# AHupuJR/REFID

Measured on AMD Instinct MI355X. Metric: interpolated frames/sec (train step) GoPro 256x256 11+1, higher is better.
Workload: dtype f32

## Files before the change

### refid_amd/csrc/conv_pw.hip

```cpp
#include "common.h"
#include "conv_args.h"
#include "conv_epilogue.h"
#include "conv_planes.h"
#include <cstdlib>

namespace {

typedef unsigned int u32x4 __attribute__((ext_vector_type(4)));
constexpr int KC = 8;
__device__ constexpr int PW_TA[6] = {0, 1, 0, 2, 0, 1};
__device__ constexpr int PW_TB[6] = {0, 0, 1, 0, 2, 1};

template <int NT, int XD, bool EX, bool SIX = false>
__global__ __launch_bounds__(256, (SIX || NT > 2) ? 3 : 4) void conv_pw_kernel(const ConvKArgs a, const PwExtra e) {
    const int lane = threadIdx.x & 63, wave = threadIdx.x >> 6;
    const int li = lane & 31, kh = lane >> 5;
    const long long npix = (long long)a.N * a.H * a.W;
    const long long p0 = ((long long)blockIdx.x * 4 + wave) * 32;
    const long long p = p0 + li;
    const int n0 = blockIdx.y * (32 * NT);

    const long long spanA = a.patchW ? (npix / a.patchW) * (long long)a.patchRow : npix * a.ldA;
    const long long spanB = a.patchW ? spanA - a.patchRow / 2 : npix * (a.inB ? a.ldB : a.ldA);
    const __amdgpu_buffer_rsrc_t rsA = __builtin_amdgcn_make_buffer_rsrc(
        const_cast<float*>(a.inA), 0, (int)min(spanA * 4, 0x7fffffffLL), 0x00020000);
    const __amdgpu_buffer_rsrc_t rsB = __builtin_amdgcn_make_buffer_rsrc(
        const_cast<float*>(a.inB ? a.inB : a.inA), 0, (int)min(spanB * 4, 0x7fffffffLL), 0x00020000);
    const __amdgpu_buffer_rsrc_t rsW = __builtin_amdgcn_make_buffer_rsrc(
        const_cast<float*>(a.w), 0, (int)min((long long)a.nchunks * a.CoutPad * KC * (SIX ? 6 : 4), 0x7fffffffLL), 0x00020000);
    const bool pok = p < npix;
    const long long pA = a.patchW ? (p / a.patchW) * a.patchRow + (p % a.patchW) * a.ldA : p * a.ldA;
    const long long pB = a.patchW ? (p / a.patchW) * a.patchRow + (p % a.patchW) * a.ldB : p * a.ldB;
    const int voA = pok ? (int)(pA * 4) + kh * 16 : OOB;
    const int voB = pok ? (int)(pB * 4) + kh * 16 : OOB;
    int voW[NT];
#pragma unroll
    for (int nt = 0; nt < NT; ++nt) {
        const int row = a.coBase + n0 + nt * 32 + li;
        voW[nt] = (row < a.CoutPad) ? (SIX ? row * 32 + kh * 16 : (row * KC + kh * 4) * 4) : OOB;
    }
    const int wChunk = a.CoutPad * KC * 4;
    const int wPlane = a.CoutPad * 32;

    f32x16 acc[NT];
#pragma unroll
    for (int nt = 0; nt < NT; ++nt)
#pragma unroll
        for (int r = 0; r < 16; ++r) acc[nt][r] = 0.f;

    auto load_x = [&](int ch) -> f32x4 {
        const int c0 = ch * KC;
        const bool fromA = c0 < a.Ca;
        const int soff = (fromA ? c0 : c0 - a.Ca) * 4;
        const int vo = (c0 + kh * 4 < a.Ctot) ? (fromA ? voA : voB) : OOB;
        const u32x4 v = fromA ? __builtin_amdgcn_raw_buffer_load_b128(rsA, vo, soff, 0)
                              : __builtin_amdgcn_raw_buffer_load_b128(rsB, vo, soff, 0);
        return __builtin_bit_cast(f32x4, v);
    };
    auto load_w = [&](int ch, f32x4 (&dst)[NT]) {
#pragma unroll
        for (int nt = 0; nt < NT; ++nt)
            dst[nt] = __builtin_bit_cast(f32x4, __builtin_amdgcn_raw_buffer_load_b128(rsW, voW[nt], ch * wChunk, 0));
    };
    auto load_w6 = [&](int c16, f32x4 (&dst)[3][NT]) {
#pragma unroll
        for (int pl = 0; pl < 3; ++pl)
#pragma unroll
            for (int nt = 0; nt < NT; ++nt)
                dst[pl][nt] = __builtin_bit_cast(f32x4, __builtin_amdgcn_raw_buffer_load_b128(rsW, voW[nt], (c16 * 3 + pl) * wPlane, 0));
    };
    auto mfma6 = [&](const f32x4& x0, const f32x4& x1, const f32x4 (&w6)[3][NT]) {
        f32x4 pl[3];
        split8<3>(x0, x1, pl);
#pragma unroll
        for (int t = 0; t < 6; ++t)
#pragma unroll
            for (int nt = 0; nt < NT; ++nt)
                acc[nt] = __builtin_amdgcn_mfma_f32_32x32x16_bf16(__builtin_bit_cast(bf16x8, w6[PW_TA[t]][nt]),
                                                                  __builtin_bit_cast(bf16x8, pl[PW_TB[t]]), acc[nt], 0, 0, 0);
    };

    f32x4 xr[2 * XD];
    f32x4 wr[SIX ? 1 : 2][NT];
    f32x4 w6[SIX ? 2 : 1][3][NT];
    const int nch = a.nchunks;
    __shared__ float sS[EX ? 128 : 1];
    bool ln_done = false;
    if constexpr (EX) {
        if (e.pool != nullptr) {
            __shared__ float sM[128], sZ[64];
            const int C = e.seC, Ch = C / 2, tid = threadIdx.x;
            const int n = (int)(((long long)blockIdx.x * 128) / e.hw);
            for (int c = tid; c < C; c += 256) {
                const float* pp = e.pool + (long long)n * e.poolParts * C + c;
                float s0 = 0.f;
                for (int r = 0; r < e.poolParts; ++r) s0 += pp[(long long)r * C];
                sM[c] = s0 * e.invHW;
            }
            __syncthreads();
            for (int j = tid; j < Ch; j += 256) {
                float z = e.seB1[j];
                for (int c = 0; c < C; ++c) z += e.seW1[j * C + c] * sM[c];
                sZ[j] = z > 0.f ? z : 0.f;
            }
            __syncthreads();
            for (int c = tid; c < C; c += 256) {
                float v = e.seB2[c];
                for (int j = 0; j < Ch; ++j) v += e.seW2[c * Ch + j] * sZ[j];
                sS[c] = 1.f / (1.f + __expf(-v));
            }
            __syncthreads();
            if (e.seS != nullptr && blockIdx.y == 0 && ((long long)blockIdx.x * 128) % e.hw == 0) {
                for (int c = tid; c < C; c += 256) { e.seM[n * C + c] = sM[c]; e.seS[n * C + c] = sS[c]; }
                for (int j = tid; j < Ch; j += 256) e.seZ1[n * Ch + j] = sZ[j];
            }
        }
        if (e.lnG != nullptr) {
#pragma unroll
            for (int j = 0; j < 2 * XD; ++j) xr[j] = (j < nch) ? load_x(j) : f32x4{0.f, 0.f, 0.f, 0.f};
            if constexpr (SIX) load_w6(0, w6[0]);
            else load_w(0, wr[0]);
            float s1 = 0.f;
#pragma unroll
            for (int j = 0; j < 2 * XD; ++j) s1 += (xr[j][0] + xr[j][1]) + (xr[j][2] + xr[j][3]);
            s1 += __shfl_xor(s1, 32, 64);
            const float mu = s1 / (float)a.Ctot;
            float s2 = 0.f;
#pragma unroll
            for (int j = 0; j < 2 * XD; ++j)
                if (j < nch) {
#pragma unroll
                    for (int k = 0; k < 4; ++k) { const float d = xr[j][k] - mu; s2 += d * d; }
                }
            s2 += __shfl_xor(s2, 32, 64);
            const float rstd = 1.f / sqrtf(s2 / (float)a.Ctot + e.lnEps);
#pragma unroll
            for (int j = 0; j < 2 * XD; ++j)
                if (j < nch) {
                    const int c = j * KC + kh * 4;
                    const f32x4 gv = *reinterpret_cast<const f32x4*>(e.lnG + c);
                    const f32x4 bv = *reinterpret_cast<const f32x4*>(e.lnB + c);
#pragma unroll
                    for (int k = 0; k < 4; ++k) xr[j][k] = (xr[j][k] - mu) * rstd * gv[k] + bv[k];
                    if (e.lnOut != nullptr && blockIdx.y == 0 && pok)
                        *reinterpret_cast<f32x4*>(e.lnOut + p * e.ldLn + c) = xr[j];
                }
            if constexpr (SIX) {
#pragma unroll
                for (int j = 0; j < 2 * XD; j += 2)
                    if (j < nch) {
                        if (j + 2 < nch) load_w6(j / 2 + 1, w6[(j / 2 + 1) & 1]);
                        mfma6(xr[j], xr[j + 1], w6[(j / 2) & 1]);
                    }
            } else {
#pragma unroll
                for (int j = 0; j < 2 * XD; ++j)
                    if (j < nch) {
                        if (j + 1 < nch) load_w(j + 1, wr[(j + 1) & 1]);
#pragma unroll
                        for (int kk = 0; kk < 4; ++kk)
#pragma unroll
                            for (int nt = 0; nt < NT; ++nt)
                                acc[nt] = __builtin_amdgcn_mfma_f32_32x32x2f32(wr[j & 1][nt][kk], xr[j][kk], acc[nt], 0, 0, 0);
                    }
            }
            ln_done = true;
        }
    }
    if (!ln_done) {
#pragma unroll
        for (int j = 0; j < XD; ++j)
            if (j < nch) xr[j] = load_x(j);
        if constexpr (SIX) load_w6(0, w6[0]);
        else load_w(0, wr[0]);
        for (int c0 = 0; c0 < nch; c0 += 2 * XD) {
#pragma unroll
            for (int j = 0; j < 2 * XD; ++j) {
                const int c = c0 + j;
                if (c < nch) {
                    if constexpr (SIX) {
                        if ((j & 1) == 0 && c + 2 < nch) load_w6(c / 2 + 1, w6[(j / 2 + 1) & 1]);
                    } else {
                        if (c + 1 < nch) load_w(c + 1, wr[(j + 1) & 1]);
                    }
                    if (c + XD < nch) xr[(j + XD) % (2 * XD)] = load_x(c + XD);
                    if constexpr (EX) {
                        if (e.pool != nullptr) {
                            const int k0 = c * KC + kh * 4;
                            const f32x4 sv = *reinterpret_cast<const f32x4*>(&sS[k0 % e.seC]);
                            xr[j] *= sv;
                            if (e.xsOut != nullptr && blockIdx.y == 0 && pok)
                                *reinterpret_cast<f32x4*>(e.xsOut + p * e.ldXs + k0) = xr[j];
                        }
                    }
                    if constexpr (SIX) {
                        if (j & 1) mfma6(xr[j - 1], xr[j], w6[(j / 2) & 1]);
                    } else {
#pragma unroll
                        for (int kk = 0; kk < 4; ++kk)
#pragma unroll
                            for (int nt = 0; nt < NT; ++nt)
                                acc[nt] = __builtin_amdgcn_mfma_f32_32x32x2f32(wr[j & 1][nt][kk], xr[j][kk], acc[nt], 0, 0, 0);
                    }
                }
            }
        }
    }

    if (a.vecOK) {
        constexpr int HN = (NT > 2) ? 2 : NT;
        constexpr int PITCH = 8 * HN + 1;
        __shared__ f32x4 sT[4][32 * PITCH];
        f32x4* t = sT[wave];
#pragma unroll
        for (int h0 = 0; h0 < NT; h0 += HN) {
            if (h0) __syncthreads();
#pragma unroll
            for (int nt = 0; nt < HN; ++nt)
#pragma unroll
                for (int g = 0; g < 4; ++g) {
                    f32x4 v;
#pragma unroll
                    for (int k = 0; k < 4; ++k) v[k] = acc[h0 + nt][4 * g + k];
                    t[li * PITCH + nt * 8 + 2 * g + kh] = v;
                }
            __syncthreads();
#pragma unroll
            for (int it = 0; it < 4 * HN; ++it) {
                const int f = it * 64 + lane;
                const int px = f / (8 * HN), c4 = f % (8 * HN);
                const long long pp = p0 + px;
                const int j0 = n0 + h0 * 32 + c4 * 4;
                if (pp >= npix || j0 >= a.Cout) continue;
                f32x4 v = t[px * PITCH + c4];
                if (a.shuffle) {
                    const int Co1 = a.Cout >> 2;
                    const unsigned qd = (unsigned)j0 / (unsigned)Co1, ch = (unsigned)j0 - qd * Co1;
                    const unsigned up = (unsigned)pp, row = up / (unsigned)a.W, x = up - row * a.W;
                    const long long op = (long long)(2 * row + (qd >> 1)) * (2 * a.W) + 2 * x + (qd & 1);
                    conv_epilogue(a, v, ch, j0, true, EpiAtOp{op, (int)ch}, false);
                    continue;
                }
                const float* res2 = nullptr;
                if constexpr (EX) {
                    if (e.res2) res2 = e.res2 + pp * e.ldR2 + j0;
                }
                conv_epilogue<true>(a, v, a.coBase + j0, j0, true, EpiAtOp{pp, j0}, false, res2);
                if constexpr (EX) {
                    if (e.out2) {
                        f32x4 gl;
#pragma unroll
                        for (int k = 0; k < 4; ++k) gl[k] = gelu_f(v[k]);
                        *reinterpret_cast<f32x4*>(e.out2 + pp * e.ldO2 + j0) = gl;
                    }
                }
            }
        }
        return;
    }
    if (!pok) return;
#pragma unroll
    for (int nt = 0; nt < NT; ++nt) {
#pragma unroll
        for (int g = 0; g < 4; ++g) {
            const int j0 = n0 + nt * 32 + 8 * g + 4 * kh;
            f32x4 v;
#pragma unroll
            for (int k = 0; k < 4; ++k) v[k] = acc[nt][4 * g + k];
            conv_epilogue<true>(a, v, a.coBase + j0, j0, false, EpiAtOp{p, j0});
        }
    }
}

}

int refid_launch_pointwise(const ConvKArgs& ka, hipStream_t st, const PwExtra* ex, int terms) {
    ConvKArgs a = ka;
    a.nchunks = cdiv(a.Ctot, KC);
    if (a.Cout % 4) a.vecOK = 0;
    const long long npix = (long long)a.N * a.H * a.W;
    const int nb = (int)((npix + 127) / 128);
    const bool six = terms == 6;
    REFID_CHECK(!a.shuffle || (a.vecOK && ex == nullptr && terms == 0 && a.mask == nullptr && a.Cout > 32 && (a.Cout / 4) % 4 == 0 &&
                               npix < 0x7fffffffLL),
                "conv2d: ConvTranspose2d on the pointwise tile needs 16-byte aligned tensors, fp32 products, no mask / fusions and "
                "at least 16 output channels");
    REFID_CHECK(a.out2 == nullptr || (a.vecOK && ex == nullptr), "conv2d: the pointwise tile's second output needs 16-byte aligned tensors and no fusions");
    REFID_CHECK(!a.patchW || (terms == 0 && ex == nullptr && a.inB != nullptr), "conv2d: the patch form of the pointwise tile has fp32 products, no fusions");
    REFID_CHECK(terms == 0 || terms == 6, "conv2d: the pointwise tile has fp32 products (0) or six bf16 products (6), got %d", terms);
    REFID_CHECK(!six || (a.Ctot % 16 == 0 && (a.inB == nullptr || a.Ca % 16 == 0) && a.Cout > 32),
                "conv2d: the six-product pointwise tile needs channel counts that are multiples of 16 and more than 32 outputs");
    if (ex != nullptr) {
        REFID_CHECK(a.vecOK && a.Cout > 32, "conv2d: pointwise fusions need 16-byte aligned tensors and more than 32 outputs");
        REFID_CHECK(!ex->lnG || (a.inB == nullptr && a.Ctot % 8 == 0 && a.Ctot <= 64 && ex->lnB),
                    "conv2d: the LayerNorm prologue needs one source of at most 64 channels (got %d)", a.Ctot);
        REFID_CHECK(!ex->pool || (ex->hw > 0 && ex->hw % 128 == 0 && ex->seC >= 8 && ex->seC <= 128 && ex->seC % 8 == 0 &&
                                  a.Ctot % ex->seC == 0 && ex->poolParts > 0 && ex->seW1 && ex->seB1 && ex->seW2 && ex->seB2 &&
                                  (!ex->seS || (ex->seM && ex->seZ1)) && !ex->lnG),
                    "conv2d: bad squeeze-excite fusion arguments (pixels per sample must be a multiple of 128)");
        if (six) hipLaunchKernelGGL((conv_pw_kernel<2, 4, true, true>), dim3(nb, cdiv(a.Cout, 64)), dim3(256), 0, st, a, *ex);
        else hipLaunchKernelGGL((conv_pw_kernel<2, 4, true>), dim3(nb, cdiv(a.Cout, 64)), dim3(256), 0, st, a, *ex);
        REFID_LAUNCH_CHECK("conv_pw/fused");
        return 0;
    }
    const PwExtra none;
    if (six) hipLaunchKernelGGL((conv_pw_kernel<2, 4, false, true>), dim3(nb, cdiv(a.Cout, 64)), dim3(256), 0, st, a, none);
    else if (a.Cout <= 32) hipLaunchKernelGGL((conv_pw_kernel<1, 8, false>), dim3(nb, 1), dim3(256), 0, st, a, none);
    else {
        static const bool nt4 = []() { const char* e = getenv("REFID_PW_NT4"); return e && e[0] == '1'; }();
        if (nt4 && a.Cout % 128 == 0)
            hipLaunchKernelGGL((conv_pw_kernel<4, 4, false>), dim3(nb, a.Cout / 128), dim3(256), 0, st, a, none);
        else
            hipLaunchKernelGGL((conv_pw_kernel<2, 4, false>), dim3(nb, cdiv(a.Cout, 64)), dim3(256), 0, st, a, none);
    }
    REFID_LAUNCH_CHECK("conv_pw");
    return 0;
}
```

Baseline: 545.6.

## Remap pointwise conv grid for XCD locality and use wave-local swizzled transpose epilogue

Replaces the 2D grid with a 1D grid whose block index is decoded so that consecutive pixel blocks land on the same XCD and all column tiles of a pixel block are adjacent. The shared-memory transpose in the epilogue now uses an XOR swizzle instead of padding, and it synchronises with a wave barrier instead of block-wide __syncthreads, since each wave only touches its own slab. Bias is hoisted into a register before the main loop, and per-item output addresses are computed incrementally through EpiSteps. It drops the NT4 environment variant, and it relies on a new ncot field and new helpers that live elsewhere.

```diff
diff --git a/refid_amd/csrc/conv_pw.hip b/refid_amd/csrc/conv_pw.hip
--- a/refid_amd/csrc/conv_pw.hip
+++ b/refid_amd/csrc/conv_pw.hip
@@ -2,7 +2,6 @@
 #include "conv_args.h"
 #include "conv_epilogue.h"
 #include "conv_planes.h"
-#include <cstdlib>
 
 namespace {
 
@@ -12,13 +11,19 @@
 __device__ constexpr int PW_TB[6] = {0, 0, 1, 0, 2, 1};
 
 template <int NT, int XD, bool EX, bool SIX = false>
-__global__ __launch_bounds__(256, (SIX || NT > 2) ? 3 : 4) void conv_pw_kernel(const ConvKArgs a, const PwExtra e) {
+__global__ __launch_bounds__(256, SIX ? 3 : 4) void conv_pw_kernel(const ConvKArgs a, const PwExtra e) {
+    static_assert(NT == 1 || NT == 2, "the transpose slab holds the wave's whole column tile in one pass");
     const int lane = threadIdx.x & 63, wave = threadIdx.x >> 6;
     const int li = lane & 31, kh = lane >> 5;
     const long long npix = (long long)a.N * a.H * a.W;
-    const long long p0 = ((long long)blockIdx.x * 4 + wave) * 32;
+    const int xcd = blockIdx.x & 7, slot = blockIdx.x >> 3;
+    const int pb = (slot / a.ncot) * 8 + xcd;
+    const long long wg0 = (long long)pb * 128;
+    if (wg0 >= npix) return;
+    const int ct = slot % a.ncot;
+    const int n0 = ct * (32 * NT);
+    const long long p0 = wg0 + wave * 32;
     const long long p = p0 + li;
-    const int n0 = blockIdx.y * (32 * NT);
 
     const long long spanA = a.patchW ? (npix / a.patchW) * (long long)a.patchRow : npix * a.ldA;
     const long long spanB = a.patchW ? spanA - a.patchRow / 2 : npix * (a.inB ? a.ldB : a.ldA);
@@ -41,6 +46,9 @@
     }
     const int wChunk = a.CoutPad * KC * 4;
     const int wPlane = a.CoutPad * 32;
+    const int c4 = lane % (8 * NT), j0 = n0 + c4 * 4;
+    f32x4 bq = {0.f, 0.f, 0.f, 0.f};
+    if (a.vecOK && a.bias && !a.shuffle && j0 < a.Cout) bq = epi_load4(a.bias + a.coBase + j0);
 
     f32x16 acc[NT];
 #pragma unroll
@@ -90,7 +98,7 @@
         if (e.pool != nullptr) {
             __shared__ float sM[128], sZ[64];
             const int C = e.seC, Ch = C / 2, tid = threadIdx.x;
-            const int n = (int)(((long long)blockIdx.x * 128) / e.hw);
+            const int n = (int)(wg0 / e.hw);
             for (int c = tid; c < C; c += 256) {
                 const float* pp = e.pool + (long long)n * e.poolParts * C + c;
                 float s0 = 0.f;
@@ -110,7 +118,7 @@
                 sS[c] = 1.f / (1.f + __expf(-v));
             }
             __syncthreads();
-            if (e.seS != nullptr && blockIdx.y == 0 && ((long long)blockIdx.x * 128) % e.hw == 0) {
+            if (e.seS != nullptr && ct == 0 && wg0 % e.hw == 0) {
                 for (int c = tid; c < C; c += 256) { e.seM[n * C + c] = sM[c]; e.seS[n * C + c] = sS[c]; }
                 for (int j = tid; j < Ch; j += 256) e.seZ1[n * Ch + j] = sZ[j];
             }
@@ -142,7 +150,7 @@
                     const f32x4 bv = *reinterpret_cast<const f32x4*>(e.lnB + c);
 #pragma unroll
                     for (int k = 0; k < 4; ++k) xr[j][k] = (xr[j][k] - mu) * rstd * gv[k] + bv[k];
-                    if (e.lnOut != nullptr && blockIdx.y == 0 && pok)
+                    if (e.lnOut != nullptr && ct == 0 && pok)
                         *reinterpret_cast<f32x4*>(e.lnOut + p * e.ldLn + c) = xr[j];
                 }
             if constexpr (SIX) {
@@ -189,7 +197,7 @@
                             const int k0 = c * KC + kh * 4;
                             const f32x4 sv = *reinterpret_cast<const f32x4*>(&sS[k0 % e.seC]);
                             xr[j] *= sv;
-                            if (e.xsOut != nullptr && blockIdx.y == 0 && pok)
+                            if (e.xsOut != nullptr && ct == 0 && pok)
                                 *reinterpret_cast<f32x4*>(e.xsOut + p * e.ldXs + k0) = xr[j];
                         }
                     }
@@ -208,52 +216,56 @@
     }
 
     if (a.vecOK) {
-        constexpr int HN = (NT > 2) ? 2 : NT;
-        constexpr int PITCH = 8 * HN + 1;
+        constexpr int PITCH = 8 * NT;
         __shared__ f32x4 sT[4][32 * PITCH];
         f32x4* t = sT[wave];
 #pragma unroll
-        for (int h0 = 0; h0 < NT; h0 += HN) {
-            if (h0) __syncthreads();
-#pragma unroll
-            for (int nt = 0; nt < HN; ++nt)
-#pragma unroll
-                for (int g = 0; g < 4; ++g) {
-                    f32x4 v;
-#pragma unroll
-                    for (int k = 0; k < 4; ++k) v[k] = acc[h0 + nt][4 * g + k];
-                    t[li * PITCH + nt * 8 + 2 * g + kh] = v;
+        for (int nt = 0; nt < NT; ++nt)
+#pragma unroll
+            for (int g = 0; g < 4; ++g) {
+                f32x4 v;
+#pragma unroll
+                for (int k = 0; k < 4; ++k) v[k] = acc[nt][4 * g + k];
+                t[li * PITCH + ((nt * 8 + 2 * g + kh) ^ (li & 7))] = v;
+            }
+        __builtin_amdgcn_fence(__ATOMIC_RELEASE, "wavefront");
+        __builtin_amdgcn_wave_barrier();
+        __builtin_amdgcn_fence(__ATOMIC_ACQUIRE, "wavefront");
+        constexpr int PPI = 8 / NT, ITEMS = 4 * NT;
+        const int px0 = lane / (8 * NT);
+        if (j0 >= a.Cout) return;
+        const EpiSteps epi(a, a.out, p0 + px0, j0, PPI, 0, true);
+        const float* res2 = nullptr;
+        float* gout2 = nullptr;
+        int res2Step = 0, gout2Step = 0;
+        if constexpr (EX) {
+            if (e.res2) { res2 = e.res2 + (p0 + px0) * e.ldR2 + j0; res2Step = PPI * e.ldR2; }
+            if (e.out2) { gout2 = e.out2 + (p0 + px0) * e.ldO2 + j0; gout2Step = PPI * e.ldO2; }
+        }
+#pragma unroll
+        for (int it = 0; it < ITEMS; ++it) {
+            const int px = it * PPI + px0;
+            const long long pp = p0 + px;
+            if (pp >= npix) continue;
+            f32x4 v = t[px * PITCH + (c4 ^ (px & 7))];
+            if (a.shuffle) {
+                const int Co1 = a.Cout >> 2;
+                const unsigned qd = (unsigned)j0 / (unsigned)Co1, ch = (unsigned)j0 - qd * Co1;
+                const unsigned up = (unsigned)pp, row = up / (unsigned)a.W, x = up - row * a.W;
+                const long long op = (long long)(2 * row + (qd >> 1)) * (2 * a.W) + 2 * x + (qd & 1);
+                conv_epilogue(a, v, ch, j0, true, EpiAtOp{op, (int)ch}, false);
+                continue;
+            }
+            if (a.bias) v += bq;
+            epi_pre(a, v);
+            epi_tail<true>(a, v, j0, true, EpiAtSteps{epi, it, 0}, false, f32x4{}, f32x4{}, res2 ? res2 + it * res2Step : nullptr);
+            if constexpr (EX) {
+                if (gout2) {
+                    f32x4 gl;
+#pragma unroll
+                    for (int k = 0; k < 4; ++k) gl[k] = gelu_f(v[k]);
+                    *reinterpret_cast<f32x4*>(gout2 + it * gout2Step) = gl;
                 }
-            __syncthreads();
-#pragma unroll
-            for (int it = 0; it < 4 * HN; ++it) {
-                const int f = it * 64 + lane;
-                const int px = f / (8 * HN), c4 = f % (8 * HN);
-                const long long pp = p0 + px;
-                const int j0 = n0 + h0 * 32 + c4 * 4;
-                if (pp >= npix || j0 >= a.Cout) continue;
-                f32x4 v = t[px * PITCH + c4];
-                if (a.shuffle) {
-                    const int Co1 = a.Cout >> 2;
-                    const unsigned qd = (unsigned)j0 / (unsigned)Co1, ch = (unsigned)j0 - qd * Co1;
-                    const unsigned up = (unsigned)pp, row = up / (unsigned)a.W, x = up - row * a.W;
-                    const long long op = (long long)(2 * row + (qd >> 1)) * (2 * a.W) + 2 * x + (qd & 1);
-                    conv_epilogue(a, v, ch, j0, true, EpiAtOp{op, (int)ch}, false);
-                    continue;
-                }
-                const float* res2 = nullptr;
-                if constexpr (EX) {
-                    if (e.res2) res2 = e.res2 + pp * e.ldR2 + j0;
-                }
-                conv_epilogue<true>(a, v, a.coBase + j0, j0, true, EpiAtOp{pp, j0}, false, res2);
-                if constexpr (EX) {
-                    if (e.out2) {
-                        f32x4 gl;
-#pragma unroll
-                        for (int k = 0; k < 4; ++k) gl[k] = gelu_f(v[k]);
-                        *reinterpret_cast<f32x4*>(e.out2 + pp * e.ldO2 + j0) = gl;
-                    }
-                }
             }
         }
         return;
@@ -263,13 +275,20 @@
     for (int nt = 0; nt < NT; ++nt) {
 #pragma unroll
         for (int g = 0; g < 4; ++g) {
-            const int j0 = n0 + nt * 32 + 8 * g + 4 * kh;
+            const int js = n0 + nt * 32 + 8 * g + 4 * kh;
             f32x4 v;
 #pragma unroll
             for (int k = 0; k < 4; ++k) v[k] = acc[nt][4 * g + k];
-            conv_epilogue<true>(a, v, a.coBase + j0, j0, false, EpiAtOp{p, j0});
-        }
-    }
+            conv_epilogue<true>(a, v, a.coBase + js, js, false, EpiAtOp{p, js});
+        }
+    }
+}
+
+template <int NT, int XD, bool EX, bool SIX>
+void pw_launch(ConvKArgs& a, const PwExtra& e, long long npix, hipStream_t st) {
+    a.ncot = cdiv(a.Cout, 32 * NT);
+    const int nb = (int)((npix + 127) / 128);
+    hipLaunchKernelGGL((conv_pw_kernel<NT, XD, EX, SIX>), dim3(round_up(nb, 8) * a.ncot), dim3(256), 0, st, a, e);
 }
 
 }
@@ -279,7 +298,6 @@
     a.nchunks = cdiv(a.Ctot, KC);
     if (a.Cout % 4) a.vecOK = 0;
     const long long npix = (long long)a.N * a.H * a.W;
-    const int nb = (int)((npix + 127) / 128);
     const bool six = terms == 6;
     REFID_CHECK(!a.shuffle || (a.vecOK && ex == nullptr && terms == 0 && a.mask == nullptr && a.Cout > 32 && (a.Cout / 4) % 4 == 0 &&
                                npix < 0x7fffffffLL),
@@ -298,21 +316,15 @@
                                   a.Ctot % ex->seC == 0 && ex->poolParts > 0 && ex->seW1 && ex->seB1 && ex->seW2 && ex->seB2 &&
                                   (!ex->seS || (ex->seM && ex->seZ1)) && !ex->lnG),
                     "conv2d: bad squeeze-excite fusion arguments (pixels per sample must be a multiple of 128)");
-        if (six) hipLaunchKernelGGL((conv_pw_kernel<2, 4, true, true>), dim3(nb, cdiv(a.Cout, 64)), dim3(256), 0, st, a, *ex);
-        else hipLaunchKernelGGL((conv_pw_kernel<2, 4, true>), dim3(nb, cdiv(a.Cout, 64)), dim3(256), 0, st, a, *ex);
+        if (six) pw_launch<2, 4, true, true>(a, *ex, npix, st);
+        else pw_launch<2, 4, true, false>(a, *ex, npix, st);
         REFID_LAUNCH_CHECK("conv_pw/fused");
         return 0;
     }
     const PwExtra none;
-    if (six) hipLaunchKernelGGL((conv_pw_kernel<2, 4, false, true>), dim3(nb, cdiv(a.Cout, 64)), dim3(256), 0, st, a, none);
-    else if (a.Cout <= 32) hipLaunchKernelGGL((conv_pw_kernel<1, 8, false>), dim3(nb, 1), dim3(256), 0, st, a, none);
-    else {
-        static const bool nt4 = []() { const char* e = getenv("REFID_PW_NT4"); return e && e[0] == '1'; }();
-        if (nt4 && a.Cout % 128 == 0)
-            hipLaunchKernelGGL((conv_pw_kernel<4, 4, false>), dim3(nb, a.Cout / 128), dim3(256), 0, st, a, none);
-        else
-            hipLaunchKernelGGL((conv_pw_kernel<2, 4, false>), dim3(nb, cdiv(a.Cout, 64)), dim3(256), 0, st, a, none);
-    }
+    if (six) pw_launch<2, 4, false, true>(a, none, npix, st);
+    else if (a.Cout <= 32) pw_launch<1, 8, false, false>(a, none, npix, st);
+    else pw_launch<2, 4, false, false>(a, none, npix, st);
     REFID_LAUNCH_CHECK("conv_pw");
     return 0;
 }
```

After: 548.5, median of 6. No clear change (+0.5%).
